# ddrainer/FloodPlanet_Code

Measured on AMD Instinct MI355X. Metric: training tiles/sec (256x256x8ch UNet), higher is better.
Workload: dtype bf16; 1 GPU; UNet depth-4 (17.27M params), 8-band 256x256 tiles, batch 16/GPU, fwd+CE(ignore_index=0)+bwd+Adam, train-mode BN; global_batch=16, parallelism=dp1

## Files before the change

floodplanet_code_amd/csrc/fu_api.hip:

```cpp
#include "../../include/floodunet.h"
#include "fu_common.h"
#include <stdlib.h>

#include <math.h>
#include <string.h>

#include <string>
#include <vector>

using namespace fu;

namespace fu {

int conv3x3_num_stat_tiles(Prec p, int B, int H, int W) {
  return p == PREC_F32 ? conv3x3_num_stat_tiles_f32(B, H, W)
                       : (p == PREC_BF16 ? conv3x3_num_stat_tiles_bf16(B, H, W) : conv3x3_num_stat_tiles_f16(B, H, W));
}
int launch_conv3x3(Prec p, const ConvIn& in, const void* wpk, const float* bias, void* dst0, int D0, void* dst1,
                   int D1, float* stats, int* n_stat_tiles, int B, int H, int W, hipStream_t s) {
  if (p == PREC_F32)
    return launch_conv3x3_f32(in, (const float*)wpk, bias, (float*)dst0, D0, (float*)dst1, D1, stats, n_stat_tiles, B,
                              H, W, s);
  if (p == PREC_BF16)
    return launch_conv3x3_bf16(in, (const bf16_t*)wpk, bias, (bf16_t*)dst0, D0, (bf16_t*)dst1, D1, stats, n_stat_tiles,
// ... 222 lines not shown
struct Fuse {
  int p_w = -1, p_b = -1, C = 0;
  void* cat = nullptr;
  void* gcat = nullptr;
  void* y = nullptr;
  void* gy = nullptr;
  float* w3 = nullptr;
  float* dw3 = nullptr;
  void* wf = nullptr;
  void* wd = nullptr;
};

struct Feat { void* y; float* a; float* b; void* gy; int C; };

struct ProfRec { int cls; double flops; hipEvent_t e0, e1; };
struct Profiler {
  bool on = false;
  std::vector<hipEvent_t> pool;
  size_t next = 0;
  std::vector<ProfRec> recs;
  bool overflow = false;
};

struct Arena {
  struct Req { void** slot; size_t bytes; };
  std::vector<Req> reqs;
  char* base = nullptr;
  size_t total = 0;
  template <typename T> void want(T** slot, size_t bytes) {
    reqs.push_back({reinterpret_cast<void**>(slot), bytes});
  }
  int commit() {
    size_t off = 0;
    for (auto& r : reqs) off += (r.bytes + 255) & ~(size_t)255;
    total = off ? off : 256;
    FU_HIP_CHECK(hipMalloc(reinterpret_cast<void**>(&base), total));
    FU_HIP_CHECK(hipMemset(base, 0, total));
    off = 0;
    for (auto& r : reqs) {
      *r.slot = base + off;
      off += (r.bytes + 255) & ~(size_t)255;
    }
    return 0;
  }
};

}

struct Dp;
struct fu_ctx {
  fu_config cfg;
  Prec prec;
  size_t esize;
  int Hs[5], Ws[5], ch[5];
  int nE = 1;
  bool fusion = false;
  int nb = 9;
  int enc_ch[FU_MAX_ENCODERS] = {0}, enc_coff[FU_MAX_ENCODERS] = {0}, cin_pad0[FU_MAX_ENCODERS] = {0};
  void* xin[FU_MAX_ENCODERS] = {nullptr};
  std::vector<ParamInfo> params;
  std::vector<BnInfo> bns;
  int64_t total_params = 0, total_bn = 0;
  std::vector<Block> blk;
  Fuse fuse[5];
  int p_outw = -1, p_outb = -1;
  float* P = nullptr;
  float* G = nullptr;
  float* RM = nullptr;
  float* RV = nullptr;
  int64_t* NBT = nullptr;
  bool packed_dirty = true;
  bool packed_eval = false;
  Arena arena;
  std::vector<void*> extra_allocs;
  float* logits = nullptr;
  float* dlogits = nullptr;
  float* dlogits_eff = nullptr;
  float* up_scale = nullptr;
  bool have_up_scale = false;
  float* stats = nullptr;
  float* bnb_part = nullptr;
  int64_t bnb_cap = 0;
  float* db_part = nullptr;
  float* db_part2 = nullptr;
  hipStream_t side = nullptr;
  hipStream_t side_lo = nullptr;
  hipStream_t side_def = nullptr;
  hipEvent_t ev_gy = nullptr, ev_wg[2] = {nullptr, nullptr}, ev_blk = nullptr;
  hipEvent_t ev_fence[2] = {nullptr, nullptr};
  int wg_parity = 0;
  int side_mode = 1;
  bool wg_pending[2] = {false, false};
  double* dscratch = nullptr;
  fu::SyncDesc sync;
  float* slab = nullptr;
  float* ce_part = nullptr;
  float* hb_part = nullptr;
  float* loss_dev = nullptr;
  float* loss_scale = nullptr;
  int* guard = nullptr;
  unsigned long long* conf_tmp = nullptr;
  int64_t* n_valid = nullptr;
  float* adam_m = nullptr;
  float* adam_v = nullptr;
  Profiler prof;
  struct Dp* dp = nullptr;
  std::vector<PackTable> pack_tabs;
  int last_batch = 0;
  bool fwd_training = false;
  bool have_loss = false;
};

namespace {

std::string dc_prefix(int i) {
  if (i == 0) return "inc.double_conv";
  if (i <= 4) return "down" + std::to_string(i) + ".maxpool_conv.1.double_conv";
  return "up" + std::to_string(i - 4) + ".conv.double_conv";
}

int add_param(fu_ctx* c, const std::string& name, std::initializer_list<int64_t> shape) {
  ParamInfo p;
  p.name = name;
  p.ndim = (int)shape.size();
  p.numel = 1;
  int k = 0;
  for (auto d : shape) { p.shape[k++] = d; p.numel *= d; }
  for (; k < 4; ++k) p.shape[k] = 1;
  p.off = c->total_params;
  c->total_params += p.numel;
  c->params.push_back(p);
  return (int)c->params.size() - 1;
}

void build_axis(int in, std::vector<int>& i0, std::vector<int>& i1, std::vector<float>& w1, std::vector<int>& bo,
                std::vector<float>& bw, bool* ok) {
  const int out = 2 * in;
  const float scale = out > 1 ? (float)(in - 1) / (float)(out - 1) : 0.f;
  i0.resize(out); i1.resize(out); w1.resize(out);
  bo.assign((size_t)in * UP_BWD_MAX, -1);
  bw.assign((size_t)in * UP_BWD_MAX, 0.f);
  std::vector<int> cnt(in, 0);
  auto push = [&](int i, int o, float w) {
    if (w == 0.f) return;
    for (int j = 0; j < cnt[i]; ++j)
      if (bo[(size_t)i * UP_BWD_MAX + j] == o) { bw[(size_t)i * UP_BWD_MAX + j] += w; return; }
    if (cnt[i] >= UP_BWD_MAX) { *ok = false; return; }
    bo[(size_t)i * UP_BWD_MAX + cnt[i]] = o;
    bw[(size_t)i * UP_BWD_MAX + cnt[i]] = w;
    cnt[i]++;
  };
  for (int o = 0; o < out; ++o) {
    const float src = scale * (float)o;
    const int a = (int)src;
    const int off = a < in - 1 ? 1 : 0;
    float l1 = src - (float)a;
    l1 = l1 < 0.f ? 0.f : (l1 > 1.f ? 1.f : l1);
    i0[o] = a; i1[o] = a + off; w1[o] = l1;
    push(a, o, 1.f - l1);
    push(a + off, o, l1);
  }
}

template <typename T>
int upload(fu_ctx* c, const std::vector<T>& v, const T** out) {
  void* d = nullptr;
  FU_HIP_CHECK(hipMalloc(&d, v.size() * sizeof(T) + 16));
  FU_HIP_CHECK(hipMemcpy(d, v.data(), v.size() * sizeof(T), hipMemcpyHostToDevice));
  c->extra_allocs.push_back(d);
  *out = (const T*)d;
  return 0;
}

int build_up_tables(fu_ctx* c, int H, int W, UpTables* t) {
  std::vector<int> yi0, yi1, xi0, xi1, ybo, xbo;
// ... 85 lines not shown
  }
  const std::string dscope = c->fusion ? "decoder." : "";
  c->p_outw = add_param(c, dscope + "outc.conv.weight", {f.n_classes, base, 1, 1});
  c->p_outb = add_param(c, dscope + "outc.conv.bias", {f.n_classes});
  return 0;
}

int alloc_workspace(fu_ctx* c) {
  const fu_config& f = c->cfg;
  const int B = f.max_batch;
  Arena& A = c->arena;
  const size_t es = c->esize;
  auto act = [&](int level, int C) { return (size_t)B * c->Hs[level] * c->Ws[level] * C * es; };
  for (int e = 0; e < c->nE; ++e) A.want(&c->xin[e], act(0, c->cin_pad0[e]));
  int64_t max_stats = 0, max_bnb = 0, max_slab = 0, max_dbp = 0;
  int max_c = 0;
  for (int i = 0; i < c->nb; ++i) {
    Block& K = c->blk[i];
    for (int j = 0; j < 2; ++j) {
      Conv& v = K.c[j];
      const int H = c->Hs[v.level], W = c->Ws[v.level];
      const int64_t npix = (int64_t)B * H * W;
      A.want(&v.y, act(v.level, v.cout));
      A.want(&v.gy, act(v.level, v.cout));
      A.want(&v.mean, v.cout * sizeof(float));
      A.want(&v.invstd, v.cout * sizeof(float));
      A.want(&v.a, v.cout * sizeof(float));
      A.want(&v.b, v.cout * sizeof(float));
      A.want(&v.coef, v.cout * 2 * sizeof(float));
      A.want(&v.fold_scale, v.cout * sizeof(float));
      A.want(&v.fold_bias, v.cout * sizeof(float));
      A.want(&v.wf, conv3x3_pack_elems(c->prec, v.cin_pad, v.cout) * es);
      if (!(K.role == 0 && j == 0)) A.want(&v.wd, conv3x3_pack_elems(c->prec, v.cin_pad, v.cout) * es);
      max_stats = std::max<int64_t>(max_stats, (int64_t)conv3x3_num_stat_tiles(c->prec, B, H, W) * v.cout * 2);
      max_bnb = std::max<int64_t>(max_bnb, bn_bwd_partial_elems(v.cout, npix));
      max_dbp = std::max<int64_t>(max_dbp, bn_bwd_partial_elems(v.cout, npix) / 2);
      max_slab = std::max<int64_t>(max_slab, conv3x3_wgrad_slab_elems(c->prec, v.cin_pad, v.cout, B, H, W));
      max_c = std::max(max_c, v.cout);
    }
    if (K.kind == BK_DOWN) {
      A.want(&K.pooled, act(K.level, K.c[0].cin_real));
      A.want(&K.g_pooled, act(K.level, K.c[0].cin_real));
    } else if (K.kind == BK_UP) {
      const int clow = K.c[0].cin_real - c->ch[K.skip];
      A.want(&K.up, act(K.level, clow));
      A.want(&K.g_up, act(K.level, clow));
      if (!f.bilinear) {
        const int H = c->Hs[K.level], W = c->Ws[K.level];
        A.want(&K.u, act(K.level, K.ct_cout));
        A.want(&K.g_u, act(K.level, K.ct_cout));
        A.want(&K.ct_w3, (size_t)9 * K.ct_cin * 4 * K.ct_cout * sizeof(float));
        A.want(&K.ct_dw3, (size_t)9 * K.ct_cin * 4 * K.ct_cout * sizeof(float));
        A.want(&K.ct_b4, (size_t)4 * K.ct_cout * sizeof(float));
        A.want(&K.ct_wf, conv3x3_pack_elems(c->prec, K.ct_cin, 4 * K.ct_cout) * es);
        A.want(&K.ct_wd, conv3x3_pack_elems(c->prec, K.ct_cin, 4 * K.ct_cout) * es);
        max_slab = std::max<int64_t>(max_slab, conv3x3_wgrad_slab_elems(c->prec, K.ct_cin, 4 * K.ct_cout, B, H / 2, W / 2));
        max_dbp = std::max<int64_t>(max_dbp, (int64_t)2048 * K.ct_cout);
      }
    }
  }
  for (int l = 0; l < 5 && c->fusion; ++l) {
    Fuse& F = c->fuse[l];
    const int Ccat = c->nE * F.C, H = c->Hs[l], W = c->Ws[l];
    A.want(&F.cat, act(l, Ccat));
    A.want(&F.gcat, act(l, Ccat));
    A.want(&F.y, act(l, F.C));
    A.want(&F.gy, act(l, F.C));
    A.want(&F.w3, (size_t)9 * Ccat * F.C * sizeof(float));
    A.want(&F.dw3, (size_t)9 * Ccat * F.C * sizeof(float));
    A.want(&F.wf, conv3x3_pack_elems(c->prec, Ccat, F.C) * es);
    A.want(&F.wd, conv3x3_pack_elems(c->prec, Ccat, F.C) * es);
    max_slab = std::max<int64_t>(max_slab, conv3x3_wgrad_slab_elems(c->prec, Ccat, F.C, B, H, W));
    max_dbp = std::max<int64_t>(max_dbp, (int64_t)2048 * F.C);
  }
  const int64_t npix0 = (int64_t)B * f.height * f.width;
  A.want(&c->logits, npix0 * f.n_classes * sizeof(float));
  A.want(&c->dlogits, npix0 * f.n_classes * sizeof(float));
  A.want(&c->dlogits_eff, npix0 * f.n_classes * sizeof(float));
  A.want(&c->up_scale, 256);
  A.want(&c->stats, max_stats * sizeof(float));
  A.want(&c->bnb_part, max_bnb * sizeof(float));
  c->bnb_cap = max_bnb;
  A.want(&c->db_part, max_dbp * sizeof(float));
  A.want(&c->db_part2, max_dbp * sizeof(float));
  A.want(&c->dscratch, reduce_scratch_elems(std::max(max_c, 64)) * sizeof(double));
  A.want(&c->slab, max_slab * sizeof(float));
  A.want(&c->ce_part, 2 * 1024 * sizeof(float));
  A.want(&c->hb_part, head_bwd_partial_elems(f.base_channels, f.n_classes) * sizeof(float));
  A.want(&c->loss_dev, 256);
  A.want(&c->loss_scale, 256);
  A.want(&c->guard, 256);
  A.want(&c->conf_tmp, 64 * sizeof(unsigned long long));
  A.want(&c->n_valid, 256);
  FU_TRY(A.commit());
  for (int i = 5 * c->nE; i < c->nb && f.bilinear; ++i) {
    Block& K = c->blk[i];
    const int lowlvl = K.level + 1;
    FU_TRY(build_up_tables(c, c->Hs[lowlvl], c->Ws[lowlvl], &K.upt));
  }
  return 0;
}

ProfSlot prof_arm(fu_ctx* c, int cls, double flops) {
  Profiler& pr = c->prof;
  ProfSlot ps;
  if (!pr.on) return ps;
  if (pr.next + 2 > pr.pool.size()) { pr.overflow = true; return ps; }
  ProfRec r{cls, flops, pr.pool[pr.next], pr.pool[pr.next + 1]};
  pr.next += 2;
  pr.recs.push_back(r);
  ps.start = r.e0;
  ps.stop = r.e1;
  return ps;
}

inline float* P(fu_ctx* c, int idx) { return c->P + c->params[idx].off; }
inline float* G(fu_ctx* c, int idx) { return c->G + c->params[idx].off; }

int repack(fu_ctx* c, hipStream_t s, bool eval) {
  if (FU_EXP_SKIP(8) && !c->pack_tabs.empty() && c->packed_eval == eval) { c->packed_dirty = false; return 0; }
  const int use_scale = eval ? 1 : 0;
  if (eval) {
    for (int i = 0; i < c->nb; ++i)
      for (int j = 0; j < 2; ++j) {
        Conv& v = c->blk[i].c[j];
        const int64_t off = c->bns[v.bn].off;
        hipLaunchKernelGGL(k_bn_fold_eval, dim3(fu::ceil_div(v.cout, 64)), dim3(64), 0, s, v.cout, P(c, v.p_g),
                           P(c, v.p_beta), c->RM + off, c->RV + off, P(c, v.p_b), BN_EPS, v.fold_scale, v.fold_bias, v.a,
                           v.b);
      }
    hipError_t e = hipGetLastError();
    if (e != hipSuccess) { set_error("eval fold launch failed: %s", hipGetErrorString(e)); return FU_ERR_HIP; }
  }
  if (c->pack_tabs.empty()) {
    bool tiled_ok = true;
    for (int i = 0; i < c->nb; ++i)
      for (int j = 0; j < 2; ++j) {
        const Conv& v = c->blk[i].c[j];
        if (v.cout % 8 != 0 || v.cin_pad % 8 != 0) tiled_ok = false;
      }
    int64_t start = 0;
    for (int i = 0; i < c->nb; ++i)
      for (int j = 0; j < 2; ++j) {
        Conv& v = c->blk[i].c[j];
        if (c->pack_tabs.empty() || c->pack_tabs.back().n == MAX_PACK) {
          PackTable nt;
          nt.n = 0; nt.total = 0; nt.tiles = 0;
          c->pack_tabs.push_back(nt);
          start = 0;
        }
        PackTable& t = c->pack_tabs.back();
        PackDesc& d = t.d[t.n++];
        d.start = start;
        d.w_off = c->params[v.p_w].off;
        d.cout = v.cout; d.cin_real = v.cin_real; d.cin_pad = v.cin_pad; d.pad_ = 0;
        d.wf = v.wf; d.wd = v.wd;
        d.scale = v.fold_scale;
        start += (int64_t)9 * v.cin_pad * v.cout;
        d.tile_start = t.tiles;
        d.tiles_ci = fu::ceil_div(v.cin_pad, 32);
        t.tiles += fu::ceil_div(v.cout, 32) * d.tiles_ci;
        t.total = start;
      }
    if (!tiled_ok) for (PackTable& t : c->pack_tabs) t.tiles = 0;
  }
  const int grid = 2048;
  for (const PackTable& t : c->pack_tabs) {
// ... 96 lines not shown
    const int64_t npix = (int64_t)B * H * W;
    int ndbp = 0;
    FU_TRY(launch_channel_partial_sums(c->prec, F.gy, F.C, npix, c->db_part, &ndbp, s));
    ConvIn in{F.cat, Ccat, nullptr, nullptr, nullptr, 0, true};
    FU_TRY(launch_conv3x3_wgrad(c->prec, in, F.gy, F.C, c->slab, F.dw3, Ccat, c->db_part, ndbp, G(c, F.p_b), B, H, W,
                                s));
    FU_TRY(launch_center_from_w3(F.dw3, (int64_t)F.C * Ccat, G(c, F.p_w), s));
    ConvIn gin{F.gy, F.C, nullptr, nullptr, nullptr, 0, true};
    if (c->nE == 2 && F.C % 64 == 0) {
      FU_TRY(launch_conv3x3(c->prec, gin, F.wd, nullptr, c->blk[l].c[1].gy, F.C, c->blk[5 + l].c[1].gy, F.C, nullptr,
                            nullptr, B, H, W, s));
    } else {
      FU_TRY(launch_conv3x3(c->prec, gin, F.wd, nullptr, F.gcat, Ccat, nullptr, 0, nullptr, nullptr, B, H, W, s));
      for (int e = 0; e < c->nE; ++e) {
        Conv& v = c->blk[5 * e + l].c[1];
        FU_TRY(launch_copy_channels(c->prec, F.gcat, Ccat, e * F.C, nullptr, nullptr, v.gy, v.cout, 0, F.C, npix, s));
      }
    }
  }
  return 0;
}

int forward_impl(fu_ctx* c, const float* x, const SrcList* srcs, int B, bool training, float* logits_out,
                 hipStream_t s) {
  const fu_config& f = c->cfg;
  if (c->packed_dirty || c->packed_eval != !training) FU_TRY(repack(c, s, !training));
  for (int e = 0; e < c->nE; ++e) {
    if (srcs)
      FU_TRY(launch_gather_nchw_to_nhwc(c->prec, *srcs, c->xin[e], B, c->enc_ch[e], f.height, f.width, c->cin_pad0[e],
                                        c->enc_coff[e], s));
    else
      FU_TRY(launch_nchw_to_nhwc(c->prec, x, c->xin[e], B, c->enc_ch[e], f.height, f.width, c->cin_pad0[e], s,
                                 f.n_channels, c->enc_coff[e]));
  }
  for (int i = 0; i < c->nb; ++i) {
    Block& K = c->blk[i];
    if (c->fusion && i == 5 * c->nE) FU_TRY(fuse_forward(c, B, s));
    if (K.kind == BK_DOWN) {
      Conv& pv = c->blk[i - 1].c[1];
      FU_TRY(launch_maxpool2(c->prec, pv.y, pv.a, pv.b, K.pooled, B, c->Hs[pv.level], c->Ws[pv.level], pv.cout, s));
    } else if (K.kind == BK_UP) {
      const Feat pv = low_feat(c, i);
      const int h = c->Hs[K.level + 1], w = c->Ws[K.level + 1], H = c->Hs[K.level], W = c->Ws[K.level];
      if (c->cfg.bilinear) {
        FU_TRY(launch_upsample2(c->prec, pv.y, pv.a, pv.b, K.up, B, h, w, pv.C, H, W, K.upt, s));
      } else {
        ConvIn lin{pv.y, pv.C, pv.a, pv.b, nullptr, 0, true};
        FU_TRY(launch_conv3x3(c->prec, lin, K.ct_wf, K.ct_b4, K.u, 4 * K.ct_cout, nullptr, 0, nullptr, nullptr, B, h, w, s));
        FU_TRY(launch_depth_to_space(c->prec, K.u, K.up, B, h, w, K.ct_cout, H, W, s));
      }
    }
    FU_TRY(conv_fwd(c, i, 0, B, training, s));
    FU_TRY(conv_fwd(c, i, 1, B, training, s));
  }
  Conv& last = c->blk[c->nb - 1].c[1];
  FU_TRY(launch_head_fwd(c->prec, last.y, last.a, last.b, P(c, c->p_outw), P(c, c->p_outb), f.base_channels,
                         f.n_classes, B, f.height, f.width, c->logits, logits_out, s));
  c->last_batch = B;
  c->fwd_training = training;
  c->have_loss = false;
  c->have_up_scale = false;
  return 0;
}

static int g_bnb_separate = getenv("FU_BNB_SEPARATE") != nullptr ? 1 : 0;
static int g_head_store_g = getenv("FU_HEAD_STORE_G") != nullptr ? 1 : 0;
static float g_test_perturb_bnb = 1.f;
__global__ void k_scale_floats(float* x, int64_t n, float f) {
  for (int64_t i = (int64_t)blockIdx.x * blockDim.x + threadIdx.x; i < n; i += (int64_t)gridDim.x * blockDim.x) x[i] *= f;
}
int perturb_bnb(float* part, int tiles, int C, hipStream_t s) {
  if (g_test_perturb_bnb == 1.f || tiles <= 0) return 0;
  hipLaunchKernelGGL(k_scale_floats, dim3(256), dim3(256), 0, s, part, (int64_t)tiles * C * 2, g_test_perturb_bnb);
  return hipGetLastError() == hipSuccess ? 0 : FU_ERR_HIP;
}

int backward_conv(fu_ctx* c, int i, int j, int B, hipStream_t s) {
  Block& K = c->blk[i];
  Conv& v = K.c[j];
  const int H = c->Hs[v.level], W = c->Ws[v.level];
  const int64_t npix = (int64_t)B * H * W;
  int ndb = 0;
  const bool side = c->side != nullptr && c->side_mode != 0;
  const int par = c->wg_parity;
  float* dbp = (side && par) ? c->db_part2 : c->db_part;
  if (side && c->wg_pending[par]) FU_HIP_CHECK(hipStreamWaitEvent(s, c->ev_wg[par], 0));
  FU_TRY(launch_bn_bwd(c->prec, v.gy, v.y, v.cout, npix, v.a, v.b, v.mean, v.invstd, P(c, v.p_g), G(c, v.p_g),
                       G(c, v.p_beta), c->bnb_part, v.coef, dbp, &ndb, c->dscratch, s, v.pool_g, B, H, W, v.bnb_tiles,
                       v.head.dl ? &v.head : nullptr));
  v.pool_g = nullptr;
  v.bnb_tiles = 0;
  v.head = HeadGrad{};
  ConvIn in = conv_input(c, i, j);
  const double fl = 2.0 * 9 * v.cin_real * v.cout * (double)B * H * W;
  hipStream_t ws = s;
  if (side) {
    FU_HIP_CHECK(hipEventRecord(c->ev_gy, s));
    FU_HIP_CHECK(hipStreamWaitEvent(c->side, c->ev_gy, 0));
    ws = c->side;
  }
  in.opt.prof = prof_arm(c, FU_K_WGRAD, fl);
  FU_TRY(launch_conv3x3_wgrad(c->prec, in, v.gy, v.cout, c->slab, G(c, v.p_w), v.cin_real, dbp, ndb,
                              G(c, v.p_b), B, H, W, ws));
  if (side) {
    FU_HIP_CHECK(hipEventRecord(c->ev_wg[par], c->side));
    c->wg_pending[par] = true;
    c->wg_parity ^= 1;
  }
  ConvIn din{v.gy, v.cout, nullptr, nullptr, nullptr, 0};
  if (!(K.role == 0 && j == 0)) din.opt.prof = prof_arm(c, FU_K_CONV3X3, fl);
  if (j == 1) {
    Conv& v0 = K.c[0];
    const bool separate = g_bnb_separate != 0;
    int tiles = 0;
    BnbFuse f;
    if (c->prec != PREC_F32 && !c->sync.hook && !separate) {
      f.y = v0.y; f.a = v0.a; f.b = v0.b; f.mean = v0.mean; f.invstd = v0.invstd;
      f.part = c->bnb_part; f.max_elems = c->bnb_cap; f.tiles_out = &tiles;
      din.opt.bnb = &f;
    }
    FU_TRY(launch_conv3x3(c->prec, din, v.wd, nullptr, v0.gy, v0.cout, nullptr, 0, nullptr, nullptr, B, H, W, s));
    v0.bnb_tiles = tiles;
    FU_TRY(perturb_bnb(c->bnb_part, tiles, v0.cout, s));
  } else if (K.kind == BK_DOWN) {
    FU_TRY(launch_conv3x3(c->prec, din, v.wd, nullptr, K.g_pooled, v.cin_real, nullptr, 0, nullptr, nullptr, B, H, W,
                          s));
    Conv& pv = c->blk[i - 1].c[1];
    pv.pool_g = K.g_pooled;
  } else if (K.kind == BK_UP) {
    const Feat sk = level_feat(c, K.skip);
    const Feat pv = low_feat(c, i);
    FU_TRY(launch_conv3x3(c->prec, din, v.wd, nullptr, sk.gy, sk.C, K.g_up, v.cin_real - sk.C, nullptr, nullptr,
                          B, H, W, s));
    const int h = c->Hs[K.level + 1], w = c->Ws[K.level + 1];
    if (c->cfg.bilinear) {
      FU_TRY(launch_upsample2_bwd(c->prec, K.g_up, pv.gy, B, h, w, pv.C, H, W, K.upt, s));
    } else {
      FU_TRY(launch_space_to_depth(c->prec, K.g_up, K.g_u, B, h, w, K.ct_cout, H, W, s));
      int ndbp = 0;
      FU_TRY(launch_channel_partial_sums(c->prec, K.g_u, K.ct_cout, (int64_t)B * h * w * 4, c->db_part, &ndbp, s));
      FU_TRY(launch_colsum_partials(c->db_part, ndbp, K.ct_cout, G(c, K.ct_b), s));
      ConvIn lin{pv.y, pv.C, pv.a, pv.b, nullptr, 0, true};
      FU_TRY(launch_conv3x3_wgrad(c->prec, lin, K.g_u, 4 * K.ct_cout, c->slab, K.ct_dw3, K.ct_cin, nullptr, 0, nullptr, B, h,
                                  w, s));
      FU_TRY(launch_convT_grad_from_w3(K.ct_dw3, K.ct_cin, K.ct_cout, G(c, K.ct_w), s));
      ConvIn gin{K.g_u, 4 * K.ct_cout, nullptr, nullptr, nullptr, 0, true};
      FU_TRY(launch_conv3x3(c->prec, gin, K.ct_wd, nullptr, pv.gy, K.ct_cin, nullptr, 0, nullptr, nullptr, B, h, w, s));
    }
  }
  return 0;
}

int num_backward_blocks(const fu_ctx* c) { return 5 + (c->fusion ? 1 : 0) + 5 * c->nE; }
int backward_block_index(const fu_ctx* c, int block) {
  if (block <= 4) return c->nb - block;
  const int k = block - 5 - (c->fusion ? 1 : 0);
  return 5 * c->nE - 1 - k;
}

int backward_block_impl(fu_ctx* c, int block, const float* dlogits_ext, hipStream_t s, bool join) {
  const fu_config& f = c->cfg;
  const int B = c->last_batch;
  if (block == 0) {
    if (dlogits_ext) {
      FU_TRY(launch_dlogits_from_nchw(dlogits_ext, c->dlogits, f.n_classes, B, f.height, f.width, s));
      c->have_up_scale = false;
    } else {
      FU_REQUIRE(c->have_loss, "fu_backward: no dlogits given and no fu_loss_* call since the last forward");
    }
    const float* dl = c->dlogits;
    if (c->prec == PREC_F16 || c->have_up_scale) {
      FU_TRY(launch_loss_grad_eff(c->dlogits, c->dlogits_eff, (int64_t)B * f.height * f.width * f.n_classes,
                                  c->have_up_scale ? c->up_scale : nullptr, c->ce_part,
                                  c->prec == PREC_F16 ? c->loss_scale : nullptr, s,
                                  c->prec == PREC_F16 ? c->guard : nullptr));
      dl = c->dlogits_eff;
    }
    Conv& last = c->blk[c->nb - 1].c[1];
    BnbFuse fz;
    int tiles = 0;
    const bool want = c->prec != PREC_F32 && !c->sync.hook && !g_bnb_separate;
    if (want) {
      fz.y = last.y; fz.a = last.a; fz.b = last.b; fz.mean = last.mean; fz.invstd = last.invstd;
      fz.part = c->bnb_part; fz.max_elems = c->bnb_cap; fz.tiles_out = &tiles;
      fz.skip_g = last.cout % 8 == 0 && 2048 % last.cout == 0 && !g_head_store_g;
    }
    FU_TRY(launch_head_bwd(c->prec, dl, last.y, last.a, last.b, P(c, c->p_outw), f.base_channels, f.n_classes,
                           (int64_t)B * f.height * f.width, last.gy, c->hb_part, G(c, c->p_outw), G(c, c->p_outb), s,
                           want ? &fz : nullptr));
    last.bnb_tiles = tiles;
    FU_REQUIRE(!(want && fz.skip_g) || tiles > 0, "head backward: the fused BatchNorm sums were refused (partials %lld floats)",
               (long long)c->bnb_cap);
    last.head = HeadGrad{};
    if (want && fz.skip_g) { last.head.dl = dl; last.head.w = P(c, c->p_outw); last.head.ncls = f.n_classes; }
    FU_TRY(perturb_bnb(c->bnb_part, tiles, last.cout, s));
    return 0;
  }
  if (c->fusion && block == 5) {
    if (c->side && c->side_mode != 0) {
      FU_HIP_CHECK(hipEventRecord(c->ev_blk, c->side));
      FU_HIP_CHECK(hipStreamWaitEvent(s, c->ev_blk, 0));
      c->wg_pending[0] = c->wg_pending[1] = false;
    }
    return fuse_backward(c, B, s);
  }
  const int i = backward_block_index(c, block);
  FU_TRY(backward_conv(c, i, 1, B, s));
  FU_TRY(backward_conv(c, i, 0, B, s));
  if (c->side && c->side_mode != 0 && join) {
    FU_HIP_CHECK(hipEventRecord(c->ev_blk, c->side));
    FU_HIP_CHECK(hipStreamWaitEvent(s, c->ev_blk, 0));
    c->wg_pending[0] = c->wg_pending[1] = false;
  }
  return 0;
}

int check_fwd_args(fu_ctx* c, const float* x, int batch) {
  FU_REQUIRE(c != nullptr, "null context");
  FU_REQUIRE(c->P && c->RM && c->RV && c->NBT, "fu_forward: buffers not bound (fu_bind_buffers)");
  FU_REQUIRE(x != nullptr, "fu_forward: null input");
  FU_REQUIRE(batch >= 1 && batch <= c->cfg.max_batch, "fu_forward: batch %d outside 1..%d", batch, c->cfg.max_batch);
  return 0;
}

double conv_flops(fu_ctx* c, bool train) {
  double fwd = 0.0, first = 0.0;
  for (int i = 0; i < c->nb; ++i)
    for (int j = 0; j < 2; ++j) {
      const Conv& v = c->blk[i].c[j];
      const double fl = 2.0 * 9 * v.cin_real * v.cout * c->Hs[v.level] * c->Ws[v.level];
      if (c->blk[i].role == 0 && j == 0) first += fl;
      fwd += fl;
    }
  for (int l = 0; l < 5 && c->fusion; ++l)
    fwd += 2.0 * c->nE * c->fuse[l].C * c->fuse[l].C * c->Hs[l] * c->Ws[l];
  if (!c->cfg.bilinear)
    for (int i = 5 * c->nE; i < c->nb; ++i) {
      const Block& K = c->blk[i];
      fwd += 2.0 * 4 * K.ct_cin * K.ct_cout * c->Hs[K.level + 1] * c->Ws[K.level + 1];
    }
  fwd += 2.0 * c->cfg.base_channels * c->cfg.n_classes * c->cfg.height * c->cfg.width;
  return train ? 3.0 * fwd - first : fwd;
}

}

extern "C" {

int fu_abi_version(void) { return FU_ABI_VERSION; }
const char* fu_last_error(void) { return get_error(); }

int fu_create(const fu_config* cfg, fu_ctx** out) {
  FU_REQUIRE(cfg && out, "fu_create: null argument");
  FU_REQUIRE(cfg->struct_size == (int32_t)sizeof(fu_config), "fu_create: fu_config size mismatch (%d vs %zu)",
             cfg->struct_size, sizeof(fu_config));
  FU_REQUIRE(cfg->n_channels >= 1 && cfg->n_channels <= 64, "n_channels must be 1..64");
  FU_REQUIRE(cfg->n_classes >= 1 && cfg->n_classes <= HEAD_MAX_CLS, "n_classes must be 1..%d", HEAD_MAX_CLS);
  const int b = cfg->base_channels;
  FU_REQUIRE(b == 4 || b == 8 || b == 16 || b == 32 || b == 64, "base_channels must be 4, 8, 16, 32 or 64");
  FU_REQUIRE(cfg->max_batch >= 1, "max_batch must be >= 1");
  FU_REQUIRE(cfg->height >= 16 && cfg->width >= 16, "tile must be at least 16x16");
  FU_REQUIRE(cfg->precision == FU_F32 || cfg->precision == FU_BF16 || cfg->precision == FU_F16, "unknown precision %d",
             cfg->precision);
  FU_REQUIRE(cfg->bilinear || b == 64, "bilinear=0 exists only at base_channels 64 (the reference's UNetDecoder "
             "channel plan is inconsistent for bilinear=False, unet.py:176-183)");
  FU_REQUIRE(cfg->precision == FU_F32 || b >= 8, "bf16 / fp16 precision needs base_channels >= 8");
  FU_REQUIRE(cfg->n_encoders >= 0 && cfg->n_encoders <= FU_MAX_ENCODERS, "n_encoders must be 0..%d", FU_MAX_ENCODERS);
  if (cfg->n_encoders >= 1) {
    FU_REQUIRE(cfg->bilinear, "late fusion exists only with bilinear upsampling (lf_model.py:38)");
    int sum = 0;
    for (int e = 0; e < cfg->n_encoders; ++e) {
      FU_REQUIRE(cfg->enc_channels[e] >= 1, "enc_channels[%d] must be >= 1", e);
      sum += cfg->enc_channels[e];
    }
    FU_REQUIRE(sum == cfg->n_channels, "enc_channels sum to %d, n_channels is %d", sum, cfg->n_channels);
  }
  FU_HIP_CHECK(hipSetDevice(cfg->device));
  fu_ctx* c = new (std::nothrow) fu_ctx();
  FU_REQUIRE(c, "out of host memory");
  c->cfg = *cfg;
  c->prec = cfg->precision == FU_F32 ? PREC_F32 : (cfg->precision == FU_BF16 ? PREC_BF16 : PREC_F16);
  c->esize = c->prec == PREC_F32 ? 4 : 2;
  int st = build_plan(c);
  if (st == 0) st = alloc_workspace(c);
  if (st == 0 && c->cfg.bilinear && c->prec != fu::PREC_F32 && !getenv("FU_NO_SIDE_STREAM")) {
    int plo = 0, phi = 0;
    (void)hipDeviceGetStreamPriorityRange(&plo, &phi);
#ifdef FU_EXPERIMENTS
    if (const char* e = getenv("FU_SIDE_CU_RESERVE")) {
      const int k = atoi(e);
      uint32_t mask[8];
      for (int w = 0; w < 8; ++w) {
        mask[w] = 0;
        for (int b = 0; b < 32; ++b) if (((w * 32 + b) % 8) >= k) mask[w] |= 1u << b;
      }
      if (hipExtStreamCreateWithCUMask(&c->side_def, 8, mask) != hipSuccess) c->side_def = nullptr;
      if (c->side_def) setenv("FU_SIDE_PRIO_DEFAULT", "1", 1);
    } else
#endif
    if (hipStreamCreateWithFlags(&c->side_def, hipStreamNonBlocking) != hipSuccess) c->side_def = nullptr;
    if (c->side_def && !getenv("FU_SIDE_PRIO_DEFAULT") &&
        hipStreamCreateWithPriority(&c->side_lo, hipStreamNonBlocking, plo) != hipSuccess)
      c->side_lo = nullptr;
    c->side = c->side_lo ? c->side_lo : c->side_def;
    if (c->side) {
      bool ok = hipEventCreateWithFlags(&c->ev_gy, hipEventDisableTiming) == hipSuccess &&
                hipEventCreateWithFlags(&c->ev_wg[0], hipEventDisableTiming) == hipSuccess &&
                hipEventCreateWithFlags(&c->ev_wg[1], hipEventDisableTiming) == hipSuccess &&
                hipEventCreateWithFlags(&c->ev_blk, hipEventDisableTiming) == hipSuccess;
      if (!ok) {
        if (c->side_lo) (void)hipStreamDestroy(c->side_lo);
        (void)hipStreamDestroy(c->side_def);
        c->side = c->side_lo = c->side_def = nullptr;
      }
    }
  }
  if (st != 0) { fu_destroy(c); return st; }
  *out = c;
  return FU_OK;
}

int fu_destroy(fu_ctx* c) {
  if (!c) return FU_OK;
  (void)hipSetDevice(c->cfg.device);
  (void)hipDeviceSynchronize();
  (void)fu_dp_destroy(c);
  for (hipEvent_t e : c->prof.pool) (void)hipEventDestroy(e);
  if (c->side) {
    if (c->side_lo) (void)hipStreamDestroy(c->side_lo);
    if (c->side_def) (void)hipStreamDestroy(c->side_def);
    for (hipEvent_t e : {c->ev_gy, c->ev_wg[0], c->ev_wg[1], c->ev_blk}) if (e) (void)hipEventDestroy(e);
  }
  for (hipEvent_t e : c->ev_fence) if (e) (void)hipEventDestroy(e);
  if (c->arena.base) (void)hipFree(c->arena.base);
  for (void* p : c->extra_allocs) (void)hipFree(p);
  delete c;
  return FU_OK;
}

int fu_num_params(const fu_ctx* c) { return c ? (int)c->params.size() : 0; }
int64_t fu_total_param_elems(const fu_ctx* c) { return c ? c->total_params : 0; }
int fu_param_info(const fu_ctx* c, int index, const char** name, int32_t* ndim, int64_t shape[4], int64_t* flat_offset) {
  FU_REQUIRE(c && index >= 0 && index < (int)c->params.size(), "fu_param_info: bad index %d", index);
  const ParamInfo& p = c->params[index];
  if (name) *name = p.name.c_str();
  if (ndim) *ndim = p.ndim;
  if (shape) for (int k = 0; k < 4; ++k) shape[k] = p.shape[k];
  if (flat_offset) *flat_offset = p.off;
  return FU_OK;
}
int fu_num_bn(const fu_ctx* c) { return c ? (int)c->bns.size() : 0; }
int64_t fu_total_bn_channels(const fu_ctx* c) { return c ? c->total_bn : 0; }
int fu_bn_info(const fu_ctx* c, int index, const char** name, int32_t* channels, int64_t* flat_offset) {
  FU_REQUIRE(c && index >= 0 && index < (int)c->bns.size(), "fu_bn_info: bad index %d", index);
  if (name) *name = c->bns[index].name.c_str();
  if (channels) *channels = c->bns[index].C;
  if (flat_offset) *flat_offset = c->bns[index].off;
  return FU_OK;
}

int fu_bind_buffers(fu_ctx* c, float* params, float* grads, float* running_mean, float* running_var,
                    int64_t* num_batches_tracked) {
  FU_REQUIRE(c && params && running_mean && running_var && num_batches_tracked, "fu_bind_buffers: null buffer");
  c->P = params; c->G = grads; c->RM = running_mean; c->RV = running_var; c->NBT = num_batches_tracked;
  c->packed_dirty = true;
  c->pack_tabs.clear();
  return FU_OK;
}
int fu_bind_adam_state(fu_ctx* c, float* exp_avg, float* exp_avg_sq) {
  FU_REQUIRE(c && exp_avg && exp_avg_sq, "fu_bind_adam_state: null argument");
  c->adam_m = exp_avg; c->adam_v = exp_avg_sq;
  return FU_OK;
}
int fu_params_changed(fu_ctx* c) {
  FU_REQUIRE(c, "null context");
  c->packed_dirty = true;
  return FU_OK;
}

namespace {
struct SyncScope {
  explicit SyncScope(const fu_ctx* c, bool on) { fu::g_sync = (on && c && c->sync.hook) ? &c->sync : nullptr; }
  ~SyncScope() { fu::g_sync = nullptr; }
};
struct UnscaleScope {
  explicit UnscaleScope(const fu_ctx* c) { fu::g_grad_unscale = (c && c->prec == PREC_F16) ? c->loss_scale + 1 : nullptr; }
  ~UnscaleScope() { fu::g_grad_unscale = nullptr; }
};
}

int fu_set_exact_sync(fu_ctx* c, fu_sync_hook hook, void* user, int world, void* exchange, int64_t exchange_bytes) {
  FU_REQUIRE(c, "null context");
  if (!hook || world <= 1) { c->sync = fu::SyncDesc(); return FU_OK; }
  if (c->prec == PREC_F16) {
    set_error("fu_set_exact_sync: the exact (SyncBN) mode is not available in fp16 precision; use bf16 or fp32");
    return FU_ERR_UNSUPPORTED;
  }
  FU_REQUIRE(exchange && exchange_bytes >= fu_exact_sync_bytes(c), "fu_set_exact_sync: exchange buffer of at least %lld bytes needed",
             (long long)fu_exact_sync_bytes(c));
  c->sync.hook = hook; c->sync.user = user; c->sync.world = world; c->sync.xbuf = exchange; c->sync.xbytes = exchange_bytes;
  return FU_OK;
}
int64_t fu_exact_sync_bytes(const fu_ctx* c) {
  if (!c) return 0;
  int max_c = 64;
  for (const BnInfo& b : c->bns) max_c = std::max(max_c, b.C);
  return std::max<int64_t>(fu::reduce_scratch_elems(max_c) * (int64_t)sizeof(double), 2 * 1024 * (int64_t)sizeof(float));
}

int fu_forward(fu_ctx* c, const float* x, int batch, int training, float* logits_out, fu_stream stream) {
  FU_TRY(check_fwd_args(c, x, batch));
  SyncScope sc(c, training != 0);
  return forward_impl(c, x, nullptr, batch, training != 0, logits_out, (hipStream_t)stream);
}
// ... 5 lines not shown
  SrcList S;
  S.n = n_src;
  int off = 0;
  for (int k = 0; k < n_src; ++k) {
    FU_REQUIRE(srcs[k] && src_channels[k] >= 1, "fu_forward_srcs: bad source %d", k);
    S.p[k] = srcs[k]; S.c[k] = src_channels[k]; S.coff[k] = off; off += src_channels[k];
  }
  S.coff[n_src] = off;
  FU_REQUIRE(off == c->cfg.n_channels, "fu_forward_srcs: the sources have %d channels in all, the model takes %d", off,
             c->cfg.n_channels);
  SyncScope sc(c, training != 0);
  return forward_impl(c, nullptr, &S, batch, training != 0, logits_out, (hipStream_t)stream);
}

int fu_loss_ce(fu_ctx* c, const int64_t* target, int ignore_index, float* loss_out, int64_t* confusion_out,
               int64_t* n_valid_out, fu_stream stream) {
  FU_REQUIRE(c && target, "fu_loss_ce: null argument");
  FU_REQUIRE(c->last_batch > 0, "fu_loss_ce: no forward pass yet");
  hipStream_t s = (hipStream_t)stream;
  SyncScope sc(c, c->fwd_training);
  const int64_t npix = (int64_t)c->last_batch * c->cfg.height * c->cfg.width;
  FU_TRY(launch_ce_loss(c->logits, target, c->cfg.n_classes, ignore_index, npix, c->ce_part,
                        loss_out ? loss_out : c->loss_dev, c->n_valid, confusion_out, n_valid_out, c->conf_tmp, s));
  if (c->fwd_training) {
    FU_TRY(launch_ce_grad(c->logits, target, c->cfg.n_classes, ignore_index, npix, c->n_valid, c->dlogits, s));
    c->have_loss = true;
    c->have_up_scale = false;
  }
  return FU_OK;
}

int fu_loss_bce_dice(fu_ctx* c, const int64_t* target, int ignore_index, float dice_weight, float* loss_out,
                     fu_stream stream) {
  FU_REQUIRE(c && target, "fu_loss_bce_dice: null argument");
  FU_REQUIRE(c->last_batch > 0, "fu_loss_bce_dice: no forward pass yet");
  hipStream_t s = (hipStream_t)stream;
  const int64_t npix = (int64_t)c->last_batch * c->cfg.height * c->cfg.width;
  FU_TRY(launch_bce_dice(c->logits, target, c->cfg.n_classes, ignore_index, npix, dice_weight, c->ce_part,
                         c->loss_dev + 8, loss_out ? loss_out : c->loss_dev, c->n_valid,
                         c->fwd_training ? c->dlogits : nullptr, s));
  if (c->fwd_training) { c->have_loss = true; c->have_up_scale = false; }
  return FU_OK;
}

int fu_scale_loss_grad(fu_ctx* c, const float* scale_dev, fu_stream stream) {
  FU_REQUIRE(c && scale_dev, "fu_scale_loss_grad: null argument");
  if (!(c->last_batch > 0 && c->fwd_training && c->have_loss)) {
    set_error("fu_scale_loss_grad: no loss gradient stored (training fu_forward + fu_loss_* first)");
    return FU_ERR_STATE;
  }
  FU_HIP_CHECK(hipMemcpyAsync(c->up_scale, scale_dev, sizeof(float), hipMemcpyDeviceToDevice, (hipStream_t)stream));
  c->have_up_scale = true;
  return FU_OK;
}

int fu_num_blocks(const fu_ctx* c) { return c ? num_backward_blocks(c) : 0; }

int fu_backward_block(fu_ctx* c, int block, const float* dlogits, fu_stream stream) {
  FU_REQUIRE(c, "null context");
  FU_REQUIRE(block >= 0 && block < num_backward_blocks(c), "fu_backward_block: block %d outside 0..%d", block,
             num_backward_blocks(c) - 1);
  if (!(c->last_batch > 0 && c->fwd_training)) {
    set_error("fu_backward: the last fu_forward was not a training forward");
    return FU_ERR_STATE;
  }
  FU_REQUIRE(c->G, "fu_backward: no gradient buffer bound");
  SyncScope sc(c, true);
  UnscaleScope us(c);
  return backward_block_impl(c, block, dlogits, (hipStream_t)stream, c->side_mode != 2);
}

int fu_set_side_stream(fu_ctx* c, int mode) {
  FU_REQUIRE(c && mode >= 0 && mode <= 2, "fu_set_side_stream: mode must be 0, 1 or 2");
  c->side_mode = mode;
  if (c->side) c->side = (mode == 2 || !c->side_lo) ? c->side_def : c->side_lo;
  return FU_OK;
}

int fu_backward_join(fu_ctx* c, fu_stream stream) {
  FU_REQUIRE(c, "null context");
  if (c->side && c->side_mode != 0) {
    FU_HIP_CHECK(hipEventRecord(c->ev_blk, c->side));
    FU_HIP_CHECK(hipStreamWaitEvent((hipStream_t)stream, c->ev_blk, 0));
    c->wg_pending[0] = c->wg_pending[1] = false;
  }
  return FU_OK;
}

int fu_backward_fence(fu_ctx* c, fu_stream stream, fu_stream waiter) {
  FU_REQUIRE(c, "null context");
  FU_REQUIRE(stream != waiter, "fu_backward_fence: the waiting stream must not be the compute stream (use fu_backward_join)");
  if (!c->ev_fence[0]) FU_HIP_CHECK(hipEventCreateWithFlags(&c->ev_fence[0], hipEventDisableTiming));
  if (!c->ev_fence[1]) FU_HIP_CHECK(hipEventCreateWithFlags(&c->ev_fence[1], hipEventDisableTiming));
  FU_HIP_CHECK(hipEventRecord(c->ev_fence[0], (hipStream_t)stream));
  FU_HIP_CHECK(hipStreamWaitEvent((hipStream_t)waiter, c->ev_fence[0], 0));
  if (c->side && c->side_mode != 0) {
    FU_HIP_CHECK(hipEventRecord(c->ev_fence[1], c->side));
    FU_HIP_CHECK(hipStreamWaitEvent((hipStream_t)waiter, c->ev_fence[1], 0));
  }
  return FU_OK;
}

int fu_backward(fu_ctx* c, const float* dlogits, fu_stream stream) {
  FU_REQUIRE(c, "null context");
  if (!(c->last_batch > 0 && c->fwd_training)) {
    set_error("fu_backward: the last fu_forward was not a training forward");
    return FU_ERR_STATE;
  }
  FU_REQUIRE(c->G, "fu_backward: no gradient buffer bound");
  SyncScope sc(c, true);
  UnscaleScope us(c);
  const int nblk = num_backward_blocks(c);
  for (int b = 0; b < nblk; ++b) FU_TRY(backward_block_impl(c, b, dlogits, (hipStream_t)stream, b == nblk - 1));
  return FU_OK;
}

int fu_block_param_range(const fu_ctx* c, int block, int64_t* flat_offset, int64_t* numel) {
  FU_REQUIRE(c && block >= 0 && block < num_backward_blocks(c), "fu_block_param_range: bad block %d", block);
  int first, count;
  if (block == 0) { first = c->p_outw; count = 2; }
  else if (c->fusion && block == 5) { first = c->fuse[0].p_w; count = 10; }
  else { const Block& K = c->blk[backward_block_index(c, block)]; first = K.first_param; count = K.num_params; }
  const ParamInfo& a = c->params[first];
  const ParamInfo& z = c->params[first + count - 1];
  if (flat_offset) *flat_offset = a.off;
  if (numel) *numel = z.off + z.numel - a.off;
  return FU_OK;
}

int fu_adam_step(fu_ctx* c, double lr, double beta1, double beta2, double eps, int64_t step, double grad_scale,
                 fu_stream stream) {
  FU_REQUIRE(c && c->P && c->G, "fu_adam_step: parameter / gradient buffers not bound");
  FU_REQUIRE(step >= 1, "fu_adam_step: step is 1-based");
  if (!c->adam_m || !c->adam_v) {
    set_error("fu_adam_step: no moment buffers bound (fu_bind_adam_state)");
    return FU_ERR_STATE;
  }
  const int* skip = nullptr;
  if (c->prec == PREC_F16) {
    FU_TRY(launch_grad_finite_check(c->G, c->total_params, c->guard, (hipStream_t)stream));
    skip = c->guard;
  }
  FU_TRY(launch_adam(c->P, c->G, c->adam_m, c->adam_v, c->total_params, lr, beta1, beta2, eps, step, grad_scale,
                     (hipStream_t)stream, skip));
  if (skip) FU_TRY(launch_guard_book(c->guard, (hipStream_t)stream));
  c->packed_dirty = true;
  return FU_OK;
}

int fu_fp16_guard_state(fu_ctx* c, int64_t* skipped_steps, int32_t* backoff_exponent) {
  FU_REQUIRE(c, "null context");
  int h[4] = {0, 0, 0, 0};
  if (c->prec == PREC_F16) FU_HIP_CHECK(hipMemcpy(h, c->guard, sizeof(h), hipMemcpyDeviceToHost));
  if (skipped_steps) *skipped_steps = h[1];
  if (backoff_exponent) *backoff_exponent = h[2];
  return FU_OK;
}

int fu_adam_scalars(double lr, double beta1, double beta2, double eps, int64_t step, double grad_scale, float out[7]) {
  FU_REQUIRE(out && step >= 1, "fu_adam_scalars: bad argument");
  adam_scalars(lr, beta1, beta2, eps, step, grad_scale, out);
  return FU_OK;
}

int fu_adam_step_dev(fu_ctx* c, const float* scalars_dev, fu_stream stream) {
  FU_REQUIRE(c && c->P && c->G && scalars_dev, "fu_adam_step_dev: parameter / gradient buffers not bound, or null scalars");
  if (!c->adam_m || !c->adam_v) {
// ... 483 lines not shown
```

Before: 3035 tiles/s.

## Replace double-buffered bias-grad partials with a ring to deepen wgrad overlap

The per-conv bias-gradient partial buffer shared between the BN backward on the main stream and the weight-gradient kernel on the side stream grows from two slots to a configurable ring (six by default, up to eight). The main stream now only waits on the side stream's event for a slot reused several convs later, so wgrad work can run further behind dgrad before it blocks. A full join is added before the transposed-conv path that reuses db_part. This costs a few more small buffers and events, and lets more side-stream work queue up and compete for compute.

```diff
diff --git a/floodplanet_code_amd/csrc/fu_api.hip b/floodplanet_code_amd/csrc/fu_api.hip
--- a/floodplanet_code_amd/csrc/fu_api.hip
+++ b/floodplanet_code_amd/csrc/fu_api.hip
@@ -328,15 +328,17 @@
   float* bnb_part = nullptr;
   int64_t bnb_cap = 0;
   float* db_part = nullptr;
-  float* db_part2 = nullptr;
+  static constexpr int DB_RING_MAX = 8;
+  float* db_ring[DB_RING_MAX] = {};
+  int db_ring_n = 6;
   hipStream_t side = nullptr;
   hipStream_t side_lo = nullptr;
   hipStream_t side_def = nullptr;
-  hipEvent_t ev_gy = nullptr, ev_wg[2] = {nullptr, nullptr}, ev_blk = nullptr;
+  hipEvent_t ev_gy = nullptr, ev_wg[DB_RING_MAX] = {}, ev_blk = nullptr;
   hipEvent_t ev_fence[2] = {nullptr, nullptr};
   int wg_parity = 0;
   int side_mode = 1;
-  bool wg_pending[2] = {false, false};
+  bool wg_pending[DB_RING_MAX] = {};
   double* dscratch = nullptr;
   fu::SyncDesc sync;
   float* slab = nullptr;
@@ -588,7 +590,8 @@
   A.want(&c->bnb_part, max_bnb * sizeof(float));
   c->bnb_cap = max_bnb;
   A.want(&c->db_part, max_dbp * sizeof(float));
-  A.want(&c->db_part2, max_dbp * sizeof(float));
+  if (const char* e = getenv("FU_DB_RING")) c->db_ring_n = std::min(std::max(atoi(e), 2), (int)fu_ctx::DB_RING_MAX);
+  for (int k = 0; k < c->db_ring_n; ++k) A.want(&c->db_ring[k], max_dbp * sizeof(float));
   A.want(&c->dscratch, reduce_scratch_elems(std::max(max_c, 64)) * sizeof(double));
   A.want(&c->slab, max_slab * sizeof(float));
   A.want(&c->ce_part, 2 * 1024 * sizeof(float));
@@ -851,8 +854,8 @@
   const int64_t npix = (int64_t)B * H * W;
   int ndb = 0;
   const bool side = c->side != nullptr && c->side_mode != 0;
-  const int par = c->wg_parity;
-  float* dbp = (side && par) ? c->db_part2 : c->db_part;
+  const int par = side ? c->wg_parity : 0;
+  float* dbp = c->db_ring[par];
   if (side && c->wg_pending[par]) FU_HIP_CHECK(hipStreamWaitEvent(s, c->ev_wg[par], 0));
   FU_TRY(launch_bn_bwd(c->prec, v.gy, v.y, v.cout, npix, v.a, v.b, v.mean, v.invstd, P(c, v.p_g), G(c, v.p_g),
                        G(c, v.p_beta), c->bnb_part, v.coef, dbp, &ndb, c->dscratch, s, v.pool_g, B, H, W, v.bnb_tiles,
@@ -874,7 +877,7 @@
   if (side) {
     FU_HIP_CHECK(hipEventRecord(c->ev_wg[par], c->side));
     c->wg_pending[par] = true;
-    c->wg_parity ^= 1;
+    c->wg_parity = (par + 1) % c->db_ring_n;
   }
   ConvIn din{v.gy, v.cout, nullptr, nullptr, nullptr, 0};
   if (!(K.role == 0 && j == 0)) din.opt.prof = prof_arm(c, FU_K_CONV3X3, fl);
@@ -905,6 +908,11 @@
     if (c->cfg.bilinear) {
       FU_TRY(launch_upsample2_bwd(c->prec, K.g_up, pv.gy, B, h, w, pv.C, H, W, K.upt, s));
     } else {
+      if (side) {
+        FU_HIP_CHECK(hipEventRecord(c->ev_blk, c->side));
+        FU_HIP_CHECK(hipStreamWaitEvent(s, c->ev_blk, 0));
+        for (bool& w : c->wg_pending) w = false;
+      }
       FU_TRY(launch_space_to_depth(c->prec, K.g_up, K.g_u, B, h, w, K.ct_cout, H, W, s));
       int ndbp = 0;
       FU_TRY(launch_channel_partial_sums(c->prec, K.g_u, K.ct_cout, (int64_t)B * h * w * 4, c->db_part, &ndbp, s));
@@ -969,7 +977,7 @@
     if (c->side && c->side_mode != 0) {
       FU_HIP_CHECK(hipEventRecord(c->ev_blk, c->side));
       FU_HIP_CHECK(hipStreamWaitEvent(s, c->ev_blk, 0));
-      c->wg_pending[0] = c->wg_pending[1] = false;
+      for (bool& w : c->wg_pending) w = false;
     }
     return fuse_backward(c, B, s);
   }
@@ -979,7 +987,7 @@
   if (c->side && c->side_mode != 0 && join) {
     FU_HIP_CHECK(hipEventRecord(c->ev_blk, c->side));
     FU_HIP_CHECK(hipStreamWaitEvent(s, c->ev_blk, 0));
-    c->wg_pending[0] = c->wg_pending[1] = false;
+    for (bool& w : c->wg_pending) w = false;
   }
   return 0;
 }
@@ -1074,9 +1082,8 @@
     c->side = c->side_lo ? c->side_lo : c->side_def;
     if (c->side) {
       bool ok = hipEventCreateWithFlags(&c->ev_gy, hipEventDisableTiming) == hipSuccess &&
-                hipEventCreateWithFlags(&c->ev_wg[0], hipEventDisableTiming) == hipSuccess &&
-                hipEventCreateWithFlags(&c->ev_wg[1], hipEventDisableTiming) == hipSuccess &&
                 hipEventCreateWithFlags(&c->ev_blk, hipEventDisableTiming) == hipSuccess;
+      for (hipEvent_t& e : c->ev_wg) ok = ok && hipEventCreateWithFlags(&e, hipEventDisableTiming) == hipSuccess;
       if (!ok) {
         if (c->side_lo) (void)hipStreamDestroy(c->side_lo);
         (void)hipStreamDestroy(c->side_def);
@@ -1098,7 +1105,8 @@
   if (c->side) {
     if (c->side_lo) (void)hipStreamDestroy(c->side_lo);
     if (c->side_def) (void)hipStreamDestroy(c->side_def);
-    for (hipEvent_t e : {c->ev_gy, c->ev_wg[0], c->ev_wg[1], c->ev_blk}) if (e) (void)hipEventDestroy(e);
+    for (hipEvent_t e : {c->ev_gy, c->ev_blk}) if (e) (void)hipEventDestroy(e);
+    for (hipEvent_t e : c->ev_wg) if (e) (void)hipEventDestroy(e);
   }
   for (hipEvent_t e : c->ev_fence) if (e) (void)hipEventDestroy(e);
   if (c->arena.base) (void)hipFree(c->arena.base);
@@ -1270,7 +1278,7 @@
   if (c->side && c->side_mode != 0) {
     FU_HIP_CHECK(hipEventRecord(c->ev_blk, c->side));
     FU_HIP_CHECK(hipStreamWaitEvent((hipStream_t)stream, c->ev_blk, 0));
-    c->wg_pending[0] = c->wg_pending[1] = false;
+    for (bool& w : c->wg_pending) w = false;
   }
   return FU_OK;
 }
```

Result: faster. 3085 tiles/s (median of 6 runs) (+1.7%).
